# petercorke/robotics-toolbox-python

Measured on AMD Instinct MI355X. Metric: configurations/sec (Panda 7-DOF fkine+jacob0), higher is better.
Workload: dtype f64

## Files before the change

robotics-toolbox-python_amd/csrc/kin_kernels.hip:

```cpp
#include "kin_reg.h"
#include "diff_device.h"
#include "servo_device.h"
#include "diff_kernel.h"
#include <algorithm>
#include <cstring>

namespace rtbhip {

#ifndef RTB_T_PLAIN_MAX_BYTES
#define RTB_T_PLAIN_MAX_BYTES (136ll << 20)
#endif
constexpr long long kPoseCacheBytes = RTB_T_PLAIN_MAX_BYTES;
constexpr int kKinPosePlain = 1;
constexpr int kKinPacked = 2;

template <bool WANT_T, bool WANT_J, bool WANT_H, bool COALESCED, class S>
__device__ __forceinline__ void kin_tiles(KinParams kp, DevChain dc, const S *__restrict__ q, S *__restrict__ T, S *__restrict__ J,
                                          double *__restrict__ H, double *lds)
{
    double *rows = lds;
    double *qs = lds + kWave * kp.stride;
    const ConstChain ops = const_view(dc);
    const int lane = threadIdx.x;
    const int64_t tiles = (kp.N + kWave - 1) / kWave;
    const int W = 6 * kp.n;

    for (int64_t tile = blockIdx.x; tile < tiles; tile += gridDim.x) {
        const int64_t cfg0 = tile * kWave;
        const int64_t cfg = cfg0 + lane;
        const int64_t left = kp.N - cfg0;
        const int ncfg = left < kWave ? (int)left : kWave;
        const bool live = lane < ncfg;

        kin_load_q(kp, q, cfg, lane, qs);
        Pose P;
        kin_walk<(WANT_J || WANT_H)>(kp, ops, lane, qs, rows, P);
        if (WANT_H) kin_hessian(kp, lane, rows, live, H + cfg * (int64_t)(kp.n * W));
        if (WANT_T && WANT_J && !WANT_H && COALESCED && (kp.pad & kKinPacked)) {
            double *rowsT = qs + kWave * kp.qw;
            if (kp.has_base) pose_premul(P, kp.base);
            pose_store16(P, [&](int k, double v) { rowsT[lane * 17 + k] = v; });
            __syncthreads();
            kin_flush_packed(rowsT, rows, kp.stride, W, ncfg, T + cfg0 * (16 + W), lane);
            __syncthreads();
            continue;
        }
        if (WANT_J) {
            if (COALESCED) {
                __syncthreads();
                kin_flush(rows, kp.stride, W, ncfg, J + cfg0 * W, lane);
            } else {
                kin_store_own(rows, kp.stride, W, live, J + cfg * W, lane);
            }
        }
        if (WANT_T) {
            if (COALESCED) __syncthreads();
            kin_stage_T(kp, lane, rows, P);
            if (COALESCED) {
                __syncthreads();
                if (kp.pad & kKinPosePlain) kin_flush<false>(rows, kp.stride, 16, ncfg, T + cfg0 * 16, lane);
                else kin_flush<true>(rows, kp.stride, 16, ncfg, T + cfg0 * 16, lane);
            } else {
                kin_store_own(rows, kp.stride, 16, live, T + cfg * 16, lane);
            }
        }
        __syncthreads();
    }
}

template <bool WANT_T, bool WANT_J, bool WANT_H, bool COALESCED>
__global__ __launch_bounds__(kWave) void k_kin(KinParams kp, DevChain dc,
                                              const double *__restrict__ q, double *__restrict__ T,
                                              double *__restrict__ J, double *__restrict__ H)
{
    extern __shared__ __attribute__((aligned(16))) double lds[];
    kin_tiles<WANT_T, WANT_J, WANT_H, COALESCED>(kp, dc, q, T, J, H, lds);
}
template <bool WANT_T, bool WANT_J>
__global__ __launch_bounds__(kWave) void k_kin_f32(KinParams kp, DevChain dc, const float *__restrict__ q, float *__restrict__ T, float *__restrict__ J)
{
    extern __shared__ __attribute__((aligned(16))) double lds[];
    kin_tiles<WANT_T, WANT_J, false, true>(kp, dc, q, T, J, (double *)nullptr, lds);
}

#ifndef RTB_REG_WAVES
#define RTB_REG_WAVES 3
#endif
template <int NJ, bool WANT_T, bool WANT_J, bool PACKED = false, SegSig SIG = 0, class S>
__device__ __forceinline__ void reg_tile(const KinParams &kp, const ConstChain &cv, const S *__restrict__ q,
                                         S *__restrict__ T, S *__restrict__ J, double *buf, int lane,
                                         int64_t tile)
{
    constexpr int W = 6 * NJ;
    const int64_t cfg0 = tile * kWave;
    const int64_t left = kp.N - cfg0;
    const int ncfg = left < kWave ? (int)left : kWave;
    Pose P;
    double jac[6 * NJ];
    reg_compute<NJ, WANT_J, SIG>(kp, cv, q, cfg0 + lane, P, jac);
    if constexpr (PACKED) {
        static_assert(!PACKED || (WANT_T && WANT_J), "packed rows carry both");
        double *bufT = buf, *bufJ = buf + kPRound * 17;
#pragma unroll
        for (int r = 0; r < kWave / kPRound; ++r) {
            if (lane / kPRound == r) reg_stage_packed<NJ>(kp, P, jac, bufT, bufJ, lane % kPRound);
            __syncthreads();
            int rows = ncfg - r * kPRound;
            rows = rows < 0 ? 0 : (rows > kPRound ? kPRound : rows);
            kin_flush_packed(bufT, bufJ, W + 1, W, rows, T + (cfg0 + r * kPRound) * (16 + W), lane);
            __syncthreads();
        }
        return;
    }
    if (WANT_T) {
        reg_stage_T(kp, P, buf, lane);
        __syncthreads();
        if (kp.pad & kKinPosePlain) kin_flush<false>(buf, 17, 16, ncfg, T + cfg0 * 16, lane);
        else kin_flush<true>(buf, 17, 16, ncfg, T + cfg0 * 16, lane);
        __syncthreads();
    }
    if (WANT_J) {
#pragma unroll
        for (int r = 0; r < kWave / kJRound; ++r) {
            if (lane / kJRound == r) reg_stage_J<NJ>(jac, buf, lane % kJRound);
            __syncthreads();
            int rows = ncfg - r * kJRound;
            rows = rows < 0 ? 0 : (rows > kJRound ? kJRound : rows);
            kin_flush(buf, W + 1, W, rows, J + (cfg0 + r * kJRound) * W, lane);
            __syncthreads();
        }
    }
}

template <int NJ, bool WANT_T, bool WANT_J, bool PACKED = false, SegSig SIG = 0>
__global__ __launch_bounds__(kWave, (NJ <= kRegMaxJoints ? RTB_REG_WAVES : 2)) void k_kin_reg(KinParams kp, DevChain dc, const double *__restrict__ q,
                                                  double *__restrict__ T, double *__restrict__ J)
{
    extern __shared__ __attribute__((aligned(16))) double buf[];
    reg_tile<NJ, WANT_T, WANT_J, PACKED, SIG>(kp, const_view(dc), q, T, J, buf, threadIdx.x, xcd_tile());
}
template <int NJ, bool WANT_T, bool WANT_J, bool PACKED = false, SegSig SIG = 0>
__global__ __launch_bounds__(kWave, (NJ <= kRegMaxJoints ? RTB_REG_WAVES : 2)) void k_kin_reg_f32(KinParams kp, DevChain dc, const float *__restrict__ q,
                                                      float *__restrict__ T, float *__restrict__ J)
{
    extern __shared__ __attribute__((aligned(16))) double buf[];
    reg_tile<NJ, WANT_T, WANT_J, PACKED, SIG>(kp, const_view(dc), q, T, J, buf, threadIdx.x, xcd_tile());
}

static int g_hess_mode = 0;

template <int NJ>
__global__ __launch_bounds__(kWave, (NJ <= kRegMaxJoints ? 2 : 1)) void k_kin_hess(KinParams kp, DevChain dc, const double *__restrict__ q,
                                                       double *__restrict__ H)
{
    extern __shared__ __attribute__((aligned(16))) double buf[];
    const ConstChain cv = const_view(dc);
    const int lane = threadIdx.x;
    const int64_t cfg0 = (int64_t)blockIdx.x * kWave;
    const int64_t left = kp.N - cfg0;
    const int ncfg = left < kWave ? (int)left : kWave;
    constexpr int W = 6 * NJ;
    {
        Pose P;
        double jac[6 * NJ];
        reg_compute<NJ, true>(kp, cv, q, cfg0 + lane, P, jac);
        double *mine = buf + lane * (W + 1);
#pragma unroll
        for (int k = 0; k < W; ++k) mine[k] = jac[k];
    }
    __syncthreads();
    double *dst = H + cfg0 * (int64_t)(NJ * W);
    hessian_run<NJ>(buf, W + 1, ncfg, lane, [&](int f, double a, double b, bool both) {
        if (both) {
            typedef double v2d __attribute__((ext_vector_type(2)));
            v2d w = {a, b};
            __builtin_nontemporal_store(w, reinterpret_cast<v2d *>(dst + f));
        } else {
            __builtin_nontemporal_store(a, dst + f);
        }
    });
}

template <int NJ, int R>
__device__ __forceinline__ void hess_tile_emit(double (&jac)[6 * NJ], double *buf, int lane, int ncfg, double *__restrict__ Hrun)
{
    constexpr int HW = NJ * 6 * NJ, S = HW | 1, G = kWave / R;
    const int grp = lane / G;
    double *mine = buf + (lane - grp * G) * S;
    for (int r = 0; r < R; ++r) {
        const int cnt = ncfg - r * G < G ? ncfg - r * G : G;
        if (cnt <= 0) break;
        if (grp == r) {
#pragma unroll
            for (int k = 0; k < 6 * NJ; ++k) asm volatile("" : "+v"(jac[k]));
            hessian_from_jacobian(NJ, [&](int k) { return jac[k]; }, [&](int idx, double v) { mine[idx] = v; });
        }
        __syncthreads();
        double *dst = Hrun + (int64_t)(r * G) * HW;
        flush_rows<HW>(buf, S, cnt, lane, [&](int f, double a, double b) {
            typedef double v2d __attribute__((ext_vector_type(2)));
            v2d w = {a, b};
            __builtin_nontemporal_store(w, reinterpret_cast<v2d *>(dst + f));
        });
        __syncthreads();
    }
}

template <int NJ, int R>
__global__ __launch_bounds__(kWave, (NJ <= kRegMaxJoints && R >= 8 ? 2 : 1)) void k_kin_hess_tile(KinParams kp, DevChain dc, const double *__restrict__ q,
                                                                                               double *__restrict__ H)
{
    extern __shared__ __attribute__((aligned(16))) double buf[];
    const ConstChain cv = const_view(dc);
    const int lane = threadIdx.x;
    const int64_t cfg0 = (int64_t)blockIdx.x * kWave;
    const int64_t left = kp.N - cfg0;
    const int ncfg = left < kWave ? (int)left : kWave;
    Pose P;
    double jac[6 * NJ];
    reg_compute<NJ, true>(kp, cv, q, cfg0 + lane, P, jac);
    hess_tile_emit<NJ, R>(jac, buf, lane, ncfg, H + cfg0 * (int64_t)(NJ * 6 * NJ));
}
template <int NJ, int R>
static hipError_t launch_hess_tile(dim3 grid, hipStream_t s, const KinParams &kp, const DevChain &dc, const double *q, double *H)
{
    const size_t lds = (size_t)(kWave / R) * ((NJ * 6 * NJ) | 1) * sizeof(double);
    auto k = k_kin_hess_tile<NJ, R>;
    if (lds > 48 * 1024) { hipError_t e = hipFuncSetAttribute((const void *)k, hipFuncAttributeMaxDynamicSharedMemorySize, (int)lds); if (e != hipSuccess) return e; }
    hipLaunchKernelGGL(k, grid, dim3(kWave), lds, s, kp, dc, q, H);
    note_launch((int)grid.x, kWave, (int)lds);
    return hipGetLastError();
}
template <int NJ>
static hipError_t launch_hess_nj(dim3 grid, hipStream_t s, const KinParams &kp, const DevChain &dc, const double *q, double *H)
{
    if (g_hess_mode == 0) return launch_hess_tile<NJ, 4>(grid, s, kp, dc, q, H);
    if (g_hess_mode == 2) return launch_hess_tile<NJ, 8>(grid, s, kp, dc, q, H);
    const size_t lds = (size_t)kWave * (6 * NJ + 1) * sizeof(double);
    hipLaunchKernelGGL((k_kin_hess<NJ>), grid, dim3(kWave), lds, s, kp, dc, q, H);
    note_launch((int)grid.x, kWave, (int)lds);
    return hipGetLastError();
}

template <int NJ, int R>
__global__ __launch_bounds__(kWave, 1) void k_hess_from_jac(const double *__restrict__ J, int64_t N, double *__restrict__ H)
{
    extern __shared__ __attribute__((aligned(16))) double buf[];
    constexpr int W = 6 * NJ;
    const int lane = threadIdx.x;
    const int64_t cfg0 = (int64_t)blockIdx.x * kWave;
    const int64_t left = N - cfg0;
    const int ncfg = left < kWave ? (int)left : kWave;
    hj_load_tile(J + cfg0 * W, W, ncfg, buf, lane);
    __syncthreads();
    double jac[W];
    const double *mine = buf + lane * (W + 1);
#pragma unroll
    for (int k = 0; k < W; ++k) jac[k] = lane < ncfg ? mine[k] : 0.0;
    __syncthreads();
    hess_tile_emit<NJ, R>(jac, buf, lane, ncfg, H + cfg0 * (int64_t)(NJ * W));
}

__global__ __launch_bounds__(kWave) void k_hess_from_jac_any(int n, const double *__restrict__ J, int64_t N, double *__restrict__ H)
{
    const int64_t cfg = (int64_t)blockIdx.x * kWave + threadIdx.x;
    if (cfg >= N) return;
    const double *Jr = J + cfg * (int64_t)(6 * n);
    double *Hr = H + cfg * (int64_t)(6 * n * n);
    hessian_from_jacobian(n, [&](int k) { return Jr[k]; }, [&](int idx, double v) { Hr[idx] = v; });
}

template <int NJ>
static hipError_t launch_hess_from_jac_nj(dim3 grid, hipStream_t s, const double *J, int64_t N, double *H)
{
    constexpr int R = 4;
    const size_t a = (size_t)(kWave / R) * ((NJ * 6 * NJ) | 1), b = (size_t)kWave * (6 * NJ + 1);
    const size_t lds = (a > b ? a : b) * sizeof(double);
    auto k = k_hess_from_jac<NJ, R>;
    if (lds > 48 * 1024) { hipError_t e = hipFuncSetAttribute((const void *)k, hipFuncAttributeMaxDynamicSharedMemorySize, (int)lds); if (e != hipSuccess) return e; }
    hipLaunchKernelGGL(k, grid, dim3(kWave), lds, s, J, N, H);
    note_launch((int)grid.x, kWave, (int)lds);
// ... 296 lines not shown
    if (g_use_reg && c->n >= 1 && c->n <= kKinRegMax) {
        const size_t rl = (size_t)reg_lds_doubles_packed(c->n) * sizeof(double);
        const SegSig sig = kin_reg_sig(c, tool);
        hipError_t e = hipSuccess;
        switch (c->n) {
        case 1: e = launch_reg_packed<1>(grid, rl, s, kp, ops, q, TJ, sig); break;
        case 2: e = launch_reg_packed<2>(grid, rl, s, kp, ops, q, TJ, sig); break;
        case 3: e = launch_reg_packed<3>(grid, rl, s, kp, ops, q, TJ, sig); break;
        case 4: e = launch_reg_packed<4>(grid, rl, s, kp, ops, q, TJ, sig); break;
        case 5: e = launch_reg_packed<5>(grid, rl, s, kp, ops, q, TJ, sig); break;
        case 6: e = launch_reg_packed<6>(grid, rl, s, kp, ops, q, TJ, sig); break;
        case 7: e = launch_reg_packed<7>(grid, rl, s, kp, ops, q, TJ, sig); break;
        case 8: e = launch_reg_packed<8>(grid, rl, s, kp, ops, q, TJ, sig); break;
        case 9: e = launch_reg_packed<9>(grid, rl, s, kp, ops, q, TJ, sig); break;
        default: e = launch_reg_packed<10>(grid, rl, s, kp, ops, q, TJ, sig); break;
        }
        note_launch((int)grid.x, kWave, (int)rl);
        if (e != hipSuccess) return hip_fail(e, "k_kin_reg (packed) launch");
        return RTBHIP_OK;
    }
    const size_t lds = kin_lds_bytes(c->n, c->q_width) + (size_t)kWave * 17 * sizeof(double);
    if (lds > 160 * 1024) { set_error("chain too large for the per-wave LDS staging"); return RTBHIP_ELIMIT; }
    hipError_t e = launch_variant<true, true, false>(true, grid, lds, s, kp, ops, q, TJ, TJ, nullptr);
    note_launch((int)grid.x, kWave, (int)lds);
    if (e != hipSuccess) return hip_fail(e, "k_kin (packed) launch");
    return RTBHIP_OK;
}
int launch_kin_packed(const Chain *c, const DevChain &ops, const double *q, int64_t N, const Affine &base,
                      const Affine &tool, int frame, double *TJ, hipStream_t s)
{
    return launch_kin_packed_s(c, ops, q, N, base, tool, frame, TJ, s);
}
int launch_kin_packed_f32(const Chain *c, const DevChain &ops, const float *q, int64_t N, const Affine &base,
                          const Affine &tool, int frame, float *TJ, hipStream_t s)
{
    return launch_kin_packed_s(c, ops, q, N, base, tool, frame, TJ, s);
}

template <class S>
static int launch_kin_s(const Chain *c, const DevChain &ops, const S *q, int64_t N, const Affine &base,
                        const Affine &tool, int frame, S *T, S *J, double *H, hipStream_t s)
{
    constexpr bool kF64 = sizeof(S) == 8;
    if (N == 0) return RTBHIP_OK;
    KinParams kp;
    kp.n = c->n;
    kp.qw = c->q_width;
    kp.stride = kin_stride(c->n);
    kp.frame = frame;
    kp.has_base = base.used;
    kp.pad = (T && J && !H && (long long)N * 16 * (long long)sizeof(S) <= kPoseCacheBytes) ? kKinPosePlain : 0;
    kp.N = N;
    for (int i = 0; i < 12; i++) kp.base[i] = base.v[i];
    chain_tail(c, tool, kp.tail);
    const int64_t tiles = (N + kWave - 1) / kWave;
    int64_t g = (tiles + g_tiles_per_wave - 1) / g_tiles_per_wave;
    if (g > 0x7fffffff) g = 0x7fffffff;
    dim3 grid((unsigned)g);
    if constexpr (kF64) {
    if (g_use_reg && H && !T && !J && c->n >= 1 && c->n <= kKinRegMax && tiles <= 0x7fffffff) {
        grid = dim3((unsigned)tiles);
        hipError_t e = hipSuccess;
        switch (c->n) {
        case 1: e = launch_hess_nj<1>(grid, s, kp, ops, q, H); break;
        case 2: e = launch_hess_nj<2>(grid, s, kp, ops, q, H); break;
        case 3: e = launch_hess_nj<3>(grid, s, kp, ops, q, H); break;
        case 4: e = launch_hess_nj<4>(grid, s, kp, ops, q, H); break;
        case 5: e = launch_hess_nj<5>(grid, s, kp, ops, q, H); break;
        case 6: e = launch_hess_nj<6>(grid, s, kp, ops, q, H); break;
        case 7: e = launch_hess_nj<7>(grid, s, kp, ops, q, H); break;
        case 8: e = launch_hess_nj<8>(grid, s, kp, ops, q, H); break;
        case 9: e = launch_hess_nj<9>(grid, s, kp, ops, q, H); break;
        default: e = launch_hess_nj<10>(grid, s, kp, ops, q, H); break;
        }
        if (e != hipSuccess) return hip_fail(e, "k_kin_hess launch");
        return RTBHIP_OK;
    }
    }
    if (g_use_reg && !H && c->n >= 1 && c->n <= kKinRegMax && tiles <= 0x7fffffff) {
        grid = dim3((unsigned)tiles);
        const size_t rl = (size_t)(J ? reg_lds_doubles(c->n) : kWave * 17) * sizeof(double);
        const SegSig sig = kin_reg_sig(c, tool);
        hipError_t e = hipSuccess;
        switch (c->n) {
        case 1: e = launch_reg<1>(grid, rl, s, kp, ops, q, T, J, sig); break;
        case 2: e = launch_reg<2>(grid, rl, s, kp, ops, q, T, J, sig); break;
        case 3: e = launch_reg<3>(grid, rl, s, kp, ops, q, T, J, sig); break;
        case 4: e = launch_reg<4>(grid, rl, s, kp, ops, q, T, J, sig); break;
        case 5: e = launch_reg<5>(grid, rl, s, kp, ops, q, T, J, sig); break;
        case 6: e = launch_reg<6>(grid, rl, s, kp, ops, q, T, J, sig); break;
        case 7: e = launch_reg<7>(grid, rl, s, kp, ops, q, T, J, sig); break;
        case 8: e = launch_reg<8>(grid, rl, s, kp, ops, q, T, J, sig); break;
        case 9: e = launch_reg<9>(grid, rl, s, kp, ops, q, T, J, sig); break;
        default: e = launch_reg<10>(grid, rl, s, kp, ops, q, T, J, sig); break;
        }
        note_launch((int)grid.x, kWave, (int)rl);
        if (e != hipSuccess) return hip_fail(e, "k_kin_reg launch");
        return RTBHIP_OK;
    }
    const size_t lds = kin_lds_bytes(c->n, c->q_width);
    if (lds > 160 * 1024) { set_error("chain too large for the per-wave LDS staging"); return RTBHIP_ELIMIT; }
    const bool co = g_coalesced != 0;
    hipError_t e;
    const bool wt = T != nullptr, wj = J != nullptr, wh = H != nullptr;
    if (wt && wj && !wh) e = launch_variant<true, true, false>(co, grid, lds, s, kp, ops, q, T, J, H);
    else if (wt && !wj && !wh) e = launch_variant<true, false, false>(co, grid, lds, s, kp, ops, q, T, J, H);
    else if (!wt && wj && !wh) e = launch_variant<false, true, false>(co, grid, lds, s, kp, ops, q, T, J, H);
    else if (kF64 && !wt && !wj && wh) { if constexpr (kF64) e = launch_variant<false, false, true>(co, grid, lds, s, kp, ops, q, T, J, H); }
    else if (kF64 && wt && wj && wh) { if constexpr (kF64) e = launch_variant<true, true, true>(co, grid, lds, s, kp, ops, q, T, J, H); }
    else { set_error("launch_kin: unsupported output combination"); return RTBHIP_EINVAL; }
    note_launch((int)grid.x, kWave, (int)lds);
    if (e != hipSuccess) return hip_fail(e, "k_kin launch");
    return RTBHIP_OK;
}
int launch_kin(const Chain *c, const DevChain &ops, const double *q, int64_t N, const Affine &base,
               const Affine &tool, int frame, double *T, double *J, double *H, hipStream_t s)
{
    return launch_kin_s(c, ops, q, N, base, tool, frame, T, J, H, s);
}
int launch_kin_f32(const Chain *c, const DevChain &ops, const float *q, int64_t N, const Affine &base,
                   const Affine &tool, int frame, float *T, float *J, hipStream_t s)
{
    return launch_kin_s(c, ops, q, N, base, tool, frame, T, J, (double *)nullptr, s);
}

constexpr int kFleetMax = 32;
struct FleetArgs {
    FleetEntry e[kFleetMax];
    int32_t count, frame;
    int64_t tiles;
    int64_t tile_base;
};

template <int CLS, bool PACKED = false>
__global__ __launch_bounds__(kWave, (CLS == 0 ? RTB_REG_WAVES : 2)) void k_fleet(FleetArgs fa)
{
    extern __shared__ __attribute__((aligned(16))) double lds[];
    const int lane = threadIdx.x;
    const int64_t gt = (int64_t)blockIdx.x + fa.tile_base;
    int ci = 0;
    for (int i = 1; i < fa.count; ++i)
        if (gt >= fa.e[i].tile0) ci = i;
    const FleetEntry &fe = fa.e[ci];
    KinParams kp;
    kp.n = fe.n; kp.qw = fe.q_width; kp.stride = fe.stride;
    kp.frame = fa.frame; kp.has_base = 0; kp.pad = PACKED ? kKinPacked : 0; kp.N = fe.N;
    const ConstChain ops = const_view(fe.dc);
    for (int k = 0; k < 9; ++k) kp.tail[k] = ops.seg[fe.n].r[k];
    for (int k = 0; k < 3; ++k) kp.tail[9 + k] = ops.seg[fe.n].t[k];
    const int64_t local = gt - fe.tile0, ctiles = (fe.N + kWave - 1) / kWave;
    const int64_t tile = (ctiles <= 0x7fffffff) ? (int64_t)xcd_tile_of((unsigned)ctiles, (unsigned)local) : local;
    if (CLS == 0) {
        switch (fe.n) {
        case 1: reg_tile<1, true, true, PACKED>(kp, ops, fe.q, fe.T, fe.J, lds, lane, tile); return;
        case 2: reg_tile<2, true, true, PACKED>(kp, ops, fe.q, fe.T, fe.J, lds, lane, tile); return;
        case 3: reg_tile<3, true, true, PACKED>(kp, ops, fe.q, fe.T, fe.J, lds, lane, tile); return;
        case 4: reg_tile<4, true, true, PACKED>(kp, ops, fe.q, fe.T, fe.J, lds, lane, tile); return;
        case 5: reg_tile<5, true, true, PACKED>(kp, ops, fe.q, fe.T, fe.J, lds, lane, tile); return;
        case 6: reg_tile<6, true, true, PACKED>(kp, ops, fe.q, fe.T, fe.J, lds, lane, tile); return;
        case 7: reg_tile<7, true, true, PACKED>(kp, ops, fe.q, fe.T, fe.J, lds, lane, tile); return;
        default: reg_tile<8, true, true, PACKED>(kp, ops, fe.q, fe.T, fe.J, lds, lane, tile); return;
        }
    } else if (CLS == 1) {
        if (fe.n == 9) reg_tile<9, true, true, PACKED>(kp, ops, fe.q, fe.T, fe.J, lds, lane, tile);
        else reg_tile<10, true, true, PACKED>(kp, ops, fe.q, fe.T, fe.J, lds, lane, tile);
        return;
    }
    double *rows = lds;
    double *qs = lds + kWave * kp.stride;
    const int64_t cfg0 = tile * kWave, cfg = cfg0 + lane;
    const int64_t left = kp.N - cfg0;
    const int ncfg = left < kWave ? (int)left : kWave;
    const int W = 6 * kp.n;
    kin_load_q(kp, fe.q, cfg, lane, qs);
    Pose P;
    kin_walk<true>(kp, ops, lane, qs, rows, P);
    if (PACKED) {
        double *rowsT = qs + kWave * kp.qw;
        pose_store16(P, [&](int k, double v) { rowsT[lane * 17 + k] = v; });
        __syncthreads();
        kin_flush_packed(rowsT, rows, kp.stride, W, ncfg, fe.T + cfg0 * (16 + W), lane);
        return;
    }
    __syncthreads();
    kin_flush(rows, kp.stride, W, ncfg, fe.J + cfg0 * W, lane);
    __syncthreads();
    kin_stage_T(kp, lane, rows, P);
    __syncthreads();
    kin_flush(rows, kp.stride, 16, ncfg, fe.T + cfg0 * 16, lane);
}

static int fleet_class_of(int n) { return n <= kRegMaxJoints ? 0 : (n <= kKinRegMax ? 1 : 2); }
static int launch_fleet_class(int cls, const std::vector<FleetEntry> &entries, int frame, hipStream_t s, bool packed);
int launch_fleet(const std::vector<FleetEntry> &all, int frame, hipStream_t s, bool packed)
{
    std::vector<FleetEntry> by[3];
    for (const FleetEntry &e : all) by[fleet_class_of(e.n)].push_back(e);
    for (int c = 0; c < 3; ++c)
        if (!by[c].empty()) { int rc = launch_fleet_class(c, by[c], frame, s, packed); if (rc != RTBHIP_OK) return rc; }
    return RTBHIP_OK;
}

template <bool PACKED>
static void fleet_go(int cls, unsigned g, size_t lds, hipStream_t s, const FleetArgs &fa)
{
    if (cls == 0) hipLaunchKernelGGL((k_fleet<0, PACKED>), dim3(g), dim3(kWave), lds, s, fa);
    else if (cls == 1) hipLaunchKernelGGL((k_fleet<1, PACKED>), dim3(g), dim3(kWave), lds, s, fa);
    else hipLaunchKernelGGL((k_fleet<2, PACKED>), dim3(g), dim3(kWave), lds, s, fa);
}
template <bool PACKED>
static const void *fleet_fn(int cls)
{
    return cls == 0 ? (const void *)k_fleet<0, PACKED> : (cls == 1 ? (const void *)k_fleet<1, PACKED> : (const void *)k_fleet<2, PACKED>);
}

static int launch_fleet_class(int cls, const std::vector<FleetEntry> &entries, int frame, hipStream_t s, bool packed)
{
    for (size_t first = 0; first < entries.size(); first += kFleetMax) {
        FleetArgs fa;
        std::memset(&fa, 0, sizeof fa);
        fa.count = (int)std::min<size_t>(kFleetMax, entries.size() - first);
        fa.frame = frame;
        size_t lds = 0;
        int64_t tiles = 0;
        for (int i = 0; i < fa.count; i++) {
            fa.e[i] = entries[first + i];
            fa.e[i].stride = kin_stride(fa.e[i].n);
            fa.e[i].tile0 = tiles;
            tiles += (fa.e[i].N + kWave - 1) / kWave;
            lds = std::max(lds, cls < 2 ? (size_t)(packed ? reg_lds_doubles_packed(fa.e[i].n) : reg_lds_doubles(fa.e[i].n)) * sizeof(double)
                                        : kin_lds_bytes(fa.e[i].n, fa.e[i].q_width) + (packed ? (size_t)kWave * 17 * sizeof(double) : 0));
        }
        fa.tiles = tiles;
        if (lds > 160 * 1024) { set_error("fleet: chain too large for LDS staging"); return RTBHIP_ELIMIT; }
        const void *kfn = packed ? fleet_fn<true>(cls) : fleet_fn<false>(cls);
        if (lds > 48 * 1024) {
            hipError_t e = hipFuncSetAttribute(kfn, hipFuncAttributeMaxDynamicSharedMemorySize, (int)lds);
            if (e != hipSuccess) return hip_fail(e, "k_fleet attr");
        }
        for (int64_t t0 = 0; t0 < tiles; t0 += 0x7fffffff) {
            const int64_t g = std::min<int64_t>(0x7fffffff, tiles - t0);
            fa.tile_base = t0;
            if (packed) fleet_go<true>(cls, (unsigned)g, lds, s, fa); else fleet_go<false>(cls, (unsigned)g, lds, s, fa);
            note_launch((int)g, kWave, (int)lds);
            hipError_t e = hipGetLastError();
            if (e != hipSuccess) return hip_fail(e, "k_fleet launch");
        }
    }
    return RTBHIP_OK;
}

template <class G>
RTB_HD void vjp_pose_pullback(const Pose &P, int has_base, const double *base , G g , double (&w)[6])
{
#pragma clang fp contract(off)
    double h[12];
#pragma unroll
    for (int i = 0; i < 3; ++i)
#pragma unroll
        for (int c = 0; c < 4; ++c)
            h[4 * i + c] = has_base ? dot3x(base[i], g(c), base[4 + i], g(4 + c), base[8 + i], g(8 + c)) : g(4 * i + c);
    w[0] = h[3]; w[1] = h[7]; w[2] = h[11];
    w[3] = (mix_pm(P.r10, h[8], P.r20, h[4]) + mix_pm(P.r11, h[9], P.r21, h[5])) + mix_pm(P.r12, h[10], P.r22, h[6]);
    w[4] = (mix_pm(P.r20, h[0], P.r00, h[8]) + mix_pm(P.r21, h[1], P.r01, h[9])) + mix_pm(P.r22, h[2], P.r02, h[10]);
    w[5] = (mix_pm(P.r00, h[4], P.r10, h[0]) + mix_pm(P.r01, h[5], P.r11, h[1])) + mix_pm(P.r02, h[6], P.r12, h[2]);
}

template <bool WANT_GJ, class JGet, class GGet, class Acc>
RTB_HD void vjp_contract(int n, const double (&w)[6], JGet J, GGet G, Acc acc)
{
#pragma clang fp contract(off)
    if (!WANT_GJ) {
#pragma unroll
        for (int k = 0; k < n; ++k)
            acc(k, dot3x(J(k), w[0], J(n + k), w[1], J(2 * n + k), w[2]) + dot3x(J(3 * n + k), w[3], J(4 * n + k), w[4], J(5 * n + k), w[5]));
        return;
    }
    double sx = w[3], sy = w[4], sz = w[5];
#pragma unroll
    for (int k = n - 1; k >= 0; --k) {
        const double vx = J(k), vy = J(n + k), vz = J(2 * n + k), ox = J(3 * n + k), oy = J(4 * n + k), oz = J(5 * n + k);
        const double gvx = G(k), gvy = G(n + k), gvz = G(2 * n + k), gwx = G(3 * n + k), gwy = G(4 * n + k), gwz = G(5 * n + k);
        sx = sx + (mix_pm(vy, gvz, vz, gvy) + mix_pm(oy, gwz, oz, gwy));
        sy = sy + (mix_pm(vz, gvx, vx, gvz) + mix_pm(oz, gwx, ox, gwz));
        sz = sz + (mix_pm(vx, gvy, vy, gvx) + mix_pm(ox, gwy, oy, gwx));
        acc(k, dot3x(ox, sx, oy, sy, oz, sz));
    }
    double ax = w[0], ay = w[1], az = w[2];
#pragma unroll
    for (int k = 0; k < n; ++k) {
        const double ox = J(3 * n + k), oy = J(4 * n + k), oz = J(5 * n + k);
        const double gvx = G(k), gvy = G(n + k), gvz = G(2 * n + k);
        acc(k, dot3x(J(k), ax, J(n + k), ay, J(2 * n + k), az));
        ax = ax + mix_pm(gvy, oz, gvz, oy);
        ay = ay + mix_pm(gvz, ox, gvx, oz);
        az = az + mix_pm(gvx, oy, gvy, ox);
    }
}

template <class S>
RTB_HD void vjp_fill(const S *__restrict__ src, int W, int cnt, double *rows, int stride, int lane)
{
    const int total = cnt * W;
    int f = 2 * lane;
    int r = f / W, e = f - r * W;
    const int da = 128 / W, db = 128 - da * W;
    for (; f < total; f += 128) {
        double a, b;
#if defined(__HIP_DEVICE_COMPILE__)
        if constexpr (sizeof(S) == 4) {
            typedef float v2f __attribute__((ext_vector_type(2)));
            typedef v2f v2f_a4 __attribute__((aligned(4)));
            const v2f v = *reinterpret_cast<const v2f_a4 *>(src + f);
            a = v.x; b = v.y;
        } else {
            typedef double v2d __attribute__((ext_vector_type(2)));
            typedef v2d v2d_a8 __attribute__((aligned(8)));
            const v2d v = *reinterpret_cast<const v2d_a8 *>(src + f);
// ... 247 lines not shown
```

robotics-toolbox-python_amd/csrc/kin_reg.h:

```cpp
#pragma once
#include "kin_tile.h"
#include "trig.h"

namespace rtbhip {

constexpr int kRegMaxJoints = 8;
constexpr int kIkMaxJoints = 16;
constexpr int kKinRegMax = 10;
#ifndef RTB_JROUND
#define RTB_JROUND 32
#endif
constexpr int kJRound = RTB_JROUND;

RTB_HD int reg_lds_doubles(int n)
{
    const int a = kJRound * (6 * n + 1), b = kWave * 17;
    return a > b ? a : b;
}

#ifndef RTB_PROUND
#define RTB_PROUND 16
#endif
constexpr int kPRound = RTB_PROUND;
RTB_HD int reg_lds_doubles_packed(int n) { return kPRound * (17 + 6 * n + 1); }

inline SegSig chain_signature(const int32_t *jmeta, int n)
{
    if (n > 8) return 0;
    SegSig s = kSegSigPresent;
    for (int j = 0; j <= n; ++j) s |= seg_sig_of(j, jm_cls(jmeta[j]), jm_tmask(jmeta[j]));
    return s;
}
constexpr SegSig kSigPandaETS = kSegSigPresent | seg_sig_of(0, kSegIdentity, 4) | seg_sig_of(1, kSegRxN, 0) | seg_sig_of(2, kSegRxP, 6) | seg_sig_of(3, kSegRxP, 1) |
                                seg_sig_of(4, kSegRxN, 7) | seg_sig_of(5, kSegRxP, 0) | seg_sig_of(6, kSegRxP, 7) | seg_sig_of(7, kSegRz, 4);
constexpr SegSig kSigPandaURDF = kSegSigPresent | seg_sig_of(0, kSegIdentity, 4) | seg_sig_of(1, kSegRxN, 0) | seg_sig_of(2, kSegRxP, 2) | seg_sig_of(3, kSegRxP, 1) |
                                 seg_sig_of(4, kSegRxN, 3) | seg_sig_of(5, kSegRxP, 0) | seg_sig_of(6, kSegRxP, 1) | seg_sig_of(7, kSegRz, 4);
constexpr SegSig kSigUR = kSegSigPresent | seg_sig_of(0, kSegIdentity, 4) | seg_sig_of(1, kSegGeneral, 2) | seg_sig_of(2, kSegIdentity, 5) | seg_sig_of(3, kSegRzP, 1) |
                          seg_sig_of(4, kSegPermA, 4) | seg_sig_of(5, kSegPermB, 4) | seg_sig_of(6, kSegGeneral, 4);
template <SegSig SIG, int J, class CV>
RTB_HD void pose_mul_seg_by_sig(Pose &P, const CV &cv) { pose_mul_seg_sig<seg_sig_cls(SIG, J), seg_sig_tm(SIG, J)>(P, cv, J); }
template <int NJ, bool WANT_J, bool PLAIN, SegSig SIG, int J, class CV>
RTB_HD void reg_walk_step(const CV &cv, Pose &P, double (&jac)[6 * NJ], const int (&jmv)[NJ], const double (&c)[NJ], const double (&s)[NJ], const double (&d)[NJ])
{
    constexpr int j = J;
    {
#if defined(__HIP_DEVICE_COMPILE__)
        CV cvj = cv;
        if (PLAIN && SIG == 0 && cv_has_trig<CV>::value && j > 0) asm volatile("" : "+s"(cvj.seg), "+v"(P.tx));
        if (j == 0) pose_from_seg(P, cvj, 0);
        else if constexpr (SIG != 0) pose_mul_seg_by_sig<SIG, J>(P, cvj);
        else pose_mul_seg<((PLAIN && cv_has_trig<CV>::value) || cv_t3fma<CV>::value)>(P, cvj, j);
#else
        if (j == 0) pose_from_seg(P, cv, 0);
        else if constexpr (SIG != 0) pose_mul_seg_by_sig<SIG, J>(P, cv);
        else pose_mul_seg<cv_t3fma<CV>::value>(P, cv, j);
#endif
        if (WANT_J) {
            jac[j] = P.tx; jac[NJ + j] = P.ty; jac[2 * NJ + j] = P.tz;
            jac[3 * NJ + j] = P.r02; jac[4 * NJ + j] = P.r12; jac[5 * NJ + j] = P.r22;
        }
        if (jm_prismatic(jmv[j])) pose_tz(P, d[j]);
        else pose_rotz(P, c[j], s[j]);
        if (SIG == 0) sched_fence();
    }
}
template <int NJ, bool WANT_J, bool PLAIN, SegSig SIG, int J = 0, class CV>
RTB_HD void reg_walk_steps(const CV &cv, Pose &P, double (&jac)[6 * NJ], const int (&jmv)[NJ], const double (&c)[NJ], const double (&s)[NJ], const double (&d)[NJ])
{
    if constexpr (J < NJ) {
        reg_walk_step<NJ, WANT_J, PLAIN, SIG, J>(cv, P, jac, jmv, c, s, d);
        reg_walk_steps<NJ, WANT_J, PLAIN, SIG, J + 1>(cv, P, jac, jmv, c, s, d);
    }
}

template <int NJ, bool WANT_J>
RTB_HD void reg_close_jacobian(const Pose &P, int frame, const int (&jmv)[NJ], double (&jac)[6 * NJ])
{
    if (WANT_J) {
#pragma clang fp contract(off)
#pragma unroll
        for (int j = 0; j < NJ; ++j) {
            double zx = jac[3 * NJ + j], zy = jac[4 * NJ + j], zz = jac[5 * NJ + j];
            if (jm_flip(jmv[j])) { zx = -zx; zy = -zy; zz = -zz; }
            double vx, vy, vz, wx, wy, wz;
            if (jm_prismatic(jmv[j])) {
                vx = zx; vy = zy; vz = zz;
                wx = 0.0; wy = 0.0; wz = 0.0;
            } else {
                const double dx = P.tx - jac[j], dy = P.ty - jac[NJ + j], dz = P.tz - jac[2 * NJ + j];
                vx = mix_pm(zy, dz, zz, dy); vy = mix_pm(zz, dx, zx, dz); vz = mix_pm(zx, dy, zy, dx);
                wx = zx; wy = zy; wz = zz;
            }
            if (frame == 1) {
                double a = vx, b = vy, e = vz;
                vx = dot3x(P.r00, a, P.r10, b, P.r20, e);
                vy = dot3x(P.r01, a, P.r11, b, P.r21, e);
                vz = dot3x(P.r02, a, P.r12, b, P.r22, e);
                a = wx; b = wy; e = wz;
                wx = dot3x(P.r00, a, P.r10, b, P.r20, e);
                wy = dot3x(P.r01, a, P.r11, b, P.r21, e);
                wz = dot3x(P.r02, a, P.r12, b, P.r22, e);
            }
            jac[j] = vx; jac[NJ + j] = vy; jac[2 * NJ + j] = vz;
            jac[3 * NJ + j] = wx; jac[4 * NJ + j] = wy; jac[5 * NJ + j] = wz;
        }
    }
}

template <int NJ, bool WANT_J, bool PLAIN = false, SegSig SIG = 0, class CV, class TL>
RTB_HD void reg_core(const CV &cv, TL tail , int frame, const double (&qv)[NJ], Pose &P,
                     double (&jac)[6 * NJ])
{
    static_assert(SIG == 0 || (PLAIN && NJ <= 8), "a structure signature goes with the straight-line walk");
    double c[NJ], s[NJ], d[NJ];
    int jmv[NJ];
    bool big = false;
#pragma unroll
    for (int j = 0; j < NJ; ++j) {
        jmv[j] = PLAIN ? 0 : cv.jmeta[j];
        d[j] = PLAIN ? qv[j] : qv[j] * (jm_flip(jmv[j]) ? -1.0 : 1.0);
    }
#pragma unroll
    for (int j = 0; j < NJ; ++j) {
        if constexpr (cv_has_trig<CV>::value) sincos_reduced_tab(d[j], s[j], c[j], cv.trig);
        else sincos_reduced(d[j], s[j], c[j]);
        big = big || !(fabs(d[j]) < kTrigFastLimit);
    }
    if (wave_any(big)) {
#pragma unroll
        for (int j = 0; j < NJ; ++j) sincos(d[j], &s[j], &c[j]);
    }
    reg_walk_steps<NJ, WANT_J, PLAIN, SIG>(cv, P, jac, jmv, c, s, d);
    if constexpr (SIG != 0) pose_mul_seg_by_sig<SIG, NJ>(P, cv);
    else pose_mul_general<((PLAIN && cv_has_trig<CV>::value) || cv_t3fma<CV>::value)>(P, [&](int k) { return tail[k]; });
    sched_fence();
    reg_close_jacobian<NJ, WANT_J>(P, frame, jmv, jac);
}

template <int NJ, bool WANT_J, SegSig SIG = 0, class CV, class S>
RTB_HD void reg_compute(const KinParams &kp, const CV &cv, const S *__restrict__ q, int64_t cfg,
                        Pose &P, double (&jac)[6 * NJ])
{
    const bool live = cfg < kp.N;
    double qv[NJ];
    if constexpr (SIG != 0) {
        const S *qrow = q + (live ? cfg : 0) * kp.qw;
        int jq[NJ];
#pragma unroll
        for (int j = 0; j < NJ; ++j) jq[j] = jm_jq(cv.jmeta[j]);
#pragma unroll
        for (int j = 0; j < NJ; ++j) qv[j] = qrow[jq[j]];
#pragma unroll
        for (int j = 0; j < NJ; ++j) qv[j] = live ? qv[j] : 0.0;
        reg_core<NJ, WANT_J, true, SIG>(cv, &cv.seg[NJ].r[0], kp.frame, qv, P, jac);
    } else {
        const S *qrow = q + cfg * kp.qw;
#pragma unroll
        for (int j = 0; j < NJ; ++j) qv[j] = live ? qrow[jm_jq(cv.jmeta[j])] : 0.0;
        reg_core<NJ, WANT_J>(cv, kp.tail, kp.frame, qv, P, jac);
    }
}

template <int NJ>
RTB_HD void reg_stage_J(const double (&jac)[6 * NJ], double *buf, int slot_lane)
{
    double *mine = buf + slot_lane * (6 * NJ + 1);
#pragma unroll
    for (int k = 0; k < 6 * NJ; ++k) mine[k] = jac[k];
}

template <int NJ>
RTB_HD void reg_stage_packed(const KinParams &kp, Pose P, const double (&jac)[6 * NJ], double *bufT, double *bufJ, int slot_lane)
{
    if (kp.has_base) pose_premul(P, kp.base);
    double *mt = bufT + slot_lane * 17;
    pose_store16(P, [&](int k, double v) { mt[k] = v; });
    double *mj = bufJ + slot_lane * (6 * NJ + 1);
#pragma unroll
    for (int k = 0; k < 6 * NJ; ++k) mj[k] = jac[k];
}

RTB_HD void reg_stage_T(const KinParams &kp, Pose P, double *buf, int lane)
{
    if (kp.has_base) pose_premul(P, kp.base);
    double *mine = buf + lane * 17;
    pose_store16(P, [&](int k, double v) { mine[k] = v; });
}

}
```

robotics-toolbox-python_amd/csrc/kin_tile.h:

```cpp
#pragma once
#include "kin_device.h"

namespace rtbhip {

struct KinParams {
    int32_t n, qw, stride, frame;
    int32_t has_base, pad;
    int64_t N;
    double base[12];
    double tail[12];
};

RTB_HD int kin_stride(int n)
{
    int s = 6 * n;
    if (s < 16) s = 16;
    return s + 1;
}
RTB_HD size_t kin_lds_bytes(int n, int qw) { return (size_t)kWave * (kin_stride(n) + qw) * sizeof(double); }

template <class S>
RTB_HD void kin_load_q(const KinParams &kp, const S *__restrict__ q, int64_t cfg, int lane,
                       double *qs)
{
    const bool live = cfg < kp.N;
    const S *src = q + cfg * kp.qw;
    int c = 0;
    for (; c + 4 <= kp.qw; c += 4) {
        double a0 = live ? src[c] : 0.0, a1 = live ? src[c + 1] : 0.0;
        double a2 = live ? src[c + 2] : 0.0, a3 = live ? src[c + 3] : 0.0;
        qs[(c + 0) * kWave + lane] = a0;
        qs[(c + 1) * kWave + lane] = a1;
        qs[(c + 2) * kWave + lane] = a2;
        qs[(c + 3) * kWave + lane] = a3;
    }
    for (; c < kp.qw; ++c) qs[c * kWave + lane] = live ? src[c] : 0.0;
}

template <bool WANT_J, class CV>
RTB_HD void kin_walk(const KinParams &kp, const CV &cv, int lane, const double *qs, double *rows, Pose &P)
{
    double *mine = rows + lane * kp.stride;
    chain_walk<WANT_J>(cv, kp.n, kp.tail, P,
                       [&](int c) { return qs[c * kWave + lane]; },
                       [&](int slot, double v) { mine[slot] = v; });
    if (WANT_J)
        jacobian_close(cv, kp.n, P, kp.frame, [&](int s) { return mine[s]; },
                       [&](int s, double v) { mine[s] = v; });
}

RTB_HD void kin_stage_T(const KinParams &kp, int lane, double *rows, Pose P)
{
    if (kp.has_base) pose_premul(P, kp.base);
    double *mine = rows + lane * kp.stride;
    pose_store16(P, [&](int k, double v) { mine[k] = v; });
}


template <bool NT>
RTB_HD void store_pair_f32(float *__restrict__ dst, double a, double b)
{
#if defined(__HIP_DEVICE_COMPILE__)
    typedef float v2f __attribute__((ext_vector_type(2)));
    typedef v2f v2f_a4 __attribute__((aligned(4)));
    v2f w = {(float)a, (float)b};
    if (NT) __builtin_nontemporal_store(w, reinterpret_cast<v2f_a4 *>(dst));
    else *reinterpret_cast<v2f_a4 *>(dst) = w;
#else
    dst[0] = (float)a;
    dst[1] = (float)b;
#endif
}

template <bool NT = true, class S>
RTB_HD void kin_flush(const double *rows, int stride, int W, int ncfg, S *__restrict__ dst,
                      int lane)
{
    const int total = ncfg * W;
    int f = 2 * lane;
    int cfg = f / W, e = f - cfg * W;
    const int da = 128 / W, db = 128 - da * W;
    for (; f < total; f += 128) {
        const double *src = rows + cfg * stride + e;
        if constexpr (sizeof(S) == 4) {
            store_pair_f32<NT>(dst + f, src[0], src[1]);
            e += db;
            cfg += da;
            if (e >= W) { e -= W; cfg += 1; }
            continue;
        }
        double2 v;
        v.x = src[0];
        v.y = src[1];
#if defined(__HIP_DEVICE_COMPILE__)
        if (NT) {
            typedef double v2d __attribute__((ext_vector_type(2)));
            v2d w = {v.x, v.y};
            __builtin_nontemporal_store(w, reinterpret_cast<v2d *>(dst + f));
        } else {
            *reinterpret_cast<double2 *>(dst + f) = v;
        }
#else
        *reinterpret_cast<double2 *>(dst + f) = v;
#endif
        e += db;
        cfg += da;
        if (e >= W) { e -= W; cfg += 1; }
    }
}

template <bool NT = true, class S>
RTB_HD void kin_flush_packed(const double *rowsT, const double *rowsJ, int strideJ, int W, int ncfg, S *__restrict__ dst, int lane)
{
    const int PW = 16 + W;
    const int total = ncfg * PW;
    int f = 2 * lane;
    int cfg = f / PW, e = f - cfg * PW;
    const int da = 128 / PW, db = 128 - da * PW;
    for (; f < total; f += 128) {
        const double *src = e < 16 ? rowsT + cfg * 17 + e : rowsJ + cfg * strideJ + (e - 16);
        if constexpr (sizeof(S) == 4) {
            store_pair_f32<NT>(dst + f, src[0], src[1]);
            e += db;
            cfg += da;
            if (e >= PW) { e -= PW; cfg += 1; }
            continue;
        }
        double2 v;
        v.x = src[0];
        v.y = src[1];
#if defined(__HIP_DEVICE_COMPILE__)
        if (NT) {
            typedef double v2d __attribute__((ext_vector_type(2)));
            v2d w = {v.x, v.y};
            __builtin_nontemporal_store(w, reinterpret_cast<v2d *>(dst + f));
        } else {
            *reinterpret_cast<double2 *>(dst + f) = v;
        }
#else
        *reinterpret_cast<double2 *>(dst + f) = v;
#endif
        e += db;
        cfg += da;
        if (e >= PW) { e -= PW; cfg += 1; }
    }
}

#if defined(__HIPCC__)
__device__ __forceinline__ void flush_run(const double *rows, int stride, int W, int ncfg, double *__restrict__ dst, int lane)
{
    const int total = ncfg * W;
    for (int f = 2 * lane; f < total; f += 2 * kWave) {
        const int r = f / W, e = f - r * W;
        const double a = rows[r * stride + e];
        if (f + 1 < total) {
            const double b = (e + 1 < W) ? rows[r * stride + e + 1] : rows[(r + 1) * stride];
            typedef double v2d __attribute__((ext_vector_type(2)));
            v2d w = {a, b};
            __builtin_nontemporal_store(w, reinterpret_cast<v2d *>(dst + f));
        } else {
            __builtin_nontemporal_store(a, dst + f);
        }
    }
}
#endif

template <class S>
RTB_HD void kin_store_own(const double *rows, int stride, int W, bool live, S *__restrict__ dst_row,
                          int lane)
{
    if (!live) return;
    const double *mine = rows + lane * stride;
    for (int e = 0; e < W; e += 2) {
        if constexpr (sizeof(S) == 4) {
            store_pair_f32<false>(dst_row + e, mine[e], mine[e + 1]);
            continue;
        }
        double2 v;
        v.x = mine[e];
        v.y = mine[e + 1];
        *reinterpret_cast<double2 *>(dst_row + e) = v;
    }
}

RTB_HD void kin_hessian(const KinParams &kp, int lane, const double *rows, bool live,
                        double *__restrict__ Hrow)
{
    if (!live) return;
    const double *mine = rows + lane * kp.stride;
    hessian_from_jacobian(kp.n, [&](int s) { return mine[s]; }, [&](int idx, double v) { Hrow[idx] = v; });
}

}
```

Before: 13.17 billion.

## Software-pipeline LDS flushes for full tiles and prefetch chain constants into SGPRs

Adds a compile-time-sized flush path for full tiles. It issues LDS reads a few pieces ahead of the nontemporal global stores, so load latency overlaps with the stores. For signature-specialised chains it also fetches the needed segment constants in two halves into pinned scalar registers before walking the joints, and touches the constant block early to warm the scalar cache. This costs SGPR pressure, more code size, and extra template instantiations. The fleet path opts out with PIPE=0.

```diff
diff --git a/robotics-toolbox-python_amd/csrc/kin_kernels.hip b/robotics-toolbox-python_amd/csrc/kin_kernels.hip
--- a/robotics-toolbox-python_amd/csrc/kin_kernels.hip
+++ b/robotics-toolbox-python_amd/csrc/kin_kernels.hip
@@ -86,7 +86,7 @@
 #ifndef RTB_REG_WAVES
 #define RTB_REG_WAVES 3
 #endif
-template <int NJ, bool WANT_T, bool WANT_J, bool PACKED = false, SegSig SIG = 0, class S>
+template <int NJ, bool WANT_T, bool WANT_J, bool PACKED = false, SegSig SIG = 0, int PIPE = 1, class S>
 __device__ __forceinline__ void reg_tile(const KinParams &kp, const ConstChain &cv, const S *__restrict__ q,
                                          S *__restrict__ T, S *__restrict__ J, double *buf, int lane,
                                          int64_t tile)
@@ -107,7 +107,7 @@
             __syncthreads();
             int rows = ncfg - r * kPRound;
             rows = rows < 0 ? 0 : (rows > kPRound ? kPRound : rows);
-            kin_flush_packed(bufT, bufJ, W + 1, W, rows, T + (cfg0 + r * kPRound) * (16 + W), lane);
+            kin_flush_packed<true, PIPE * kPRound, W>(bufT, bufJ, W + 1, W, rows, T + (cfg0 + r * kPRound) * (16 + W), lane);
             __syncthreads();
         }
         return;
@@ -115,8 +115,8 @@
     if (WANT_T) {
         reg_stage_T(kp, P, buf, lane);
         __syncthreads();
-        if (kp.pad & kKinPosePlain) kin_flush<false>(buf, 17, 16, ncfg, T + cfg0 * 16, lane);
-        else kin_flush<true>(buf, 17, 16, ncfg, T + cfg0 * 16, lane);
+        if (kp.pad & kKinPosePlain) kin_flush<false, PIPE * kWave, 16>(buf, 17, 16, ncfg, T + cfg0 * 16, lane);
+        else kin_flush<true, PIPE * kWave, 16>(buf, 17, 16, ncfg, T + cfg0 * 16, lane);
         __syncthreads();
     }
     if (WANT_J) {
@@ -126,7 +126,7 @@
             __syncthreads();
             int rows = ncfg - r * kJRound;
             rows = rows < 0 ? 0 : (rows > kJRound ? kJRound : rows);
-            kin_flush(buf, W + 1, W, rows, J + (cfg0 + r * kJRound) * W, lane);
+            kin_flush<true, PIPE * kJRound, W>(buf, W + 1, W, rows, J + (cfg0 + r * kJRound) * W, lane);
             __syncthreads();
         }
     }
@@ -729,18 +729,18 @@
     const int64_t tile = (ctiles <= 0x7fffffff) ? (int64_t)xcd_tile_of((unsigned)ctiles, (unsigned)local) : local;
     if (CLS == 0) {
         switch (fe.n) {
-        case 1: reg_tile<1, true, true, PACKED>(kp, ops, fe.q, fe.T, fe.J, lds, lane, tile); return;
-        case 2: reg_tile<2, true, true, PACKED>(kp, ops, fe.q, fe.T, fe.J, lds, lane, tile); return;
-        case 3: reg_tile<3, true, true, PACKED>(kp, ops, fe.q, fe.T, fe.J, lds, lane, tile); return;
-        case 4: reg_tile<4, true, true, PACKED>(kp, ops, fe.q, fe.T, fe.J, lds, lane, tile); return;
-        case 5: reg_tile<5, true, true, PACKED>(kp, ops, fe.q, fe.T, fe.J, lds, lane, tile); return;
-        case 6: reg_tile<6, true, true, PACKED>(kp, ops, fe.q, fe.T, fe.J, lds, lane, tile); return;
-        case 7: reg_tile<7, true, true, PACKED>(kp, ops, fe.q, fe.T, fe.J, lds, lane, tile); return;
-        default: reg_tile<8, true, true, PACKED>(kp, ops, fe.q, fe.T, fe.J, lds, lane, tile); return;
+        case 1: reg_tile<1, true, true, PACKED, 0, 0>(kp, ops, fe.q, fe.T, fe.J, lds, lane, tile); return;
+        case 2: reg_tile<2, true, true, PACKED, 0, 0>(kp, ops, fe.q, fe.T, fe.J, lds, lane, tile); return;
+        case 3: reg_tile<3, true, true, PACKED, 0, 0>(kp, ops, fe.q, fe.T, fe.J, lds, lane, tile); return;
+        case 4: reg_tile<4, true, true, PACKED, 0, 0>(kp, ops, fe.q, fe.T, fe.J, lds, lane, tile); return;
+        case 5: reg_tile<5, true, true, PACKED, 0, 0>(kp, ops, fe.q, fe.T, fe.J, lds, lane, tile); return;
+        case 6: reg_tile<6, true, true, PACKED, 0, 0>(kp, ops, fe.q, fe.T, fe.J, lds, lane, tile); return;
+        case 7: reg_tile<7, true, true, PACKED, 0, 0>(kp, ops, fe.q, fe.T, fe.J, lds, lane, tile); return;
+        default: reg_tile<8, true, true, PACKED, 0, 0>(kp, ops, fe.q, fe.T, fe.J, lds, lane, tile); return;
         }
     } else if (CLS == 1) {
-        if (fe.n == 9) reg_tile<9, true, true, PACKED>(kp, ops, fe.q, fe.T, fe.J, lds, lane, tile);
-        else reg_tile<10, true, true, PACKED>(kp, ops, fe.q, fe.T, fe.J, lds, lane, tile);
+        if (fe.n == 9) reg_tile<9, true, true, PACKED, 0, 0>(kp, ops, fe.q, fe.T, fe.J, lds, lane, tile);
+        else reg_tile<10, true, true, PACKED, 0, 0>(kp, ops, fe.q, fe.T, fe.J, lds, lane, tile);
         return;
     }
     double *rows = lds;
diff --git a/robotics-toolbox-python_amd/csrc/kin_reg.h b/robotics-toolbox-python_amd/csrc/kin_reg.h
--- a/robotics-toolbox-python_amd/csrc/kin_reg.h
+++ b/robotics-toolbox-python_amd/csrc/kin_reg.h
@@ -64,12 +64,12 @@
         if (SIG == 0) sched_fence();
     }
 }
-template <int NJ, bool WANT_J, bool PLAIN, SegSig SIG, int J = 0, class CV>
+template <int NJ, bool WANT_J, bool PLAIN, SegSig SIG, int J = 0, int JEND = NJ, class CV>
 RTB_HD void reg_walk_steps(const CV &cv, Pose &P, double (&jac)[6 * NJ], const int (&jmv)[NJ], const double (&c)[NJ], const double (&s)[NJ], const double (&d)[NJ])
 {
-    if constexpr (J < NJ) {
+    if constexpr (J < JEND) {
         reg_walk_step<NJ, WANT_J, PLAIN, SIG, J>(cv, P, jac, jmv, c, s, d);
-        reg_walk_steps<NJ, WANT_J, PLAIN, SIG, J + 1>(cv, P, jac, jmv, c, s, d);
+        reg_walk_steps<NJ, WANT_J, PLAIN, SIG, J + 1, JEND>(cv, P, jac, jmv, c, s, d);
     }
 }
 
@@ -107,6 +107,83 @@
     }
 }
 
+template <int NJ>
+struct SigSegs {
+    DevSeg seg[NJ + 1];
+    const int32_t *jmeta;
+};
+constexpr bool sig_reads_entry(SegSig sig, int j, int k )
+{
+    const int cls = seg_sig_cls(sig, j), tm = seg_sig_tm(sig, j);
+    if (j == 0 || cls == kSegGeneral || ((RTB_SIG_UNFUSED_GENERAL >> cls) & 1)) return true;
+    return k < 9 ? seg_kind(cls, k) == kCA : ((tm >> (k - 9)) & 1) != 0;
+}
+constexpr int sig_reads_count(SegSig sig, int j0, int j1, int k1 = 0)
+{
+    int m = 0;
+    for (int a = j0; a <= j1; ++a)
+        for (int b = 0; b < (a < j1 ? 12 : k1); ++b) m += sig_reads_entry(sig, a, b) ? 1 : 0;
+    return m;
+}
+constexpr int kSigFetchMax = 40;
+constexpr int sig_split(SegSig sig, int nj)
+{
+    int h = 1;
+    while (h <= nj && 2 * sig_reads_count(sig, 0, h) < sig_reads_count(sig, 0, nj + 1)) ++h;
+    return h;
+}
+constexpr bool sig_fetches(SegSig sig, int nj)
+{
+    if (sig == 0 || nj > 8) return false;
+    const int h = sig_split(sig, nj);
+    return sig_reads_count(sig, 0, nj + 1) <= kSigFetchMax && sig_reads_count(sig, 0, h) <= 30 && sig_reads_count(sig, h, nj + 1) <= 30;
+}
+template <int V> struct IntC { static constexpr int v = V; };
+template <SegSig SIG, int J0, int J1, int I = 12 * J0, class F>
+RTB_HD void sig_each(F f)
+{
+    if constexpr (I < 12 * J1) {
+        if constexpr (sig_reads_entry(SIG, I / 12, I % 12)) f(IntC<I / 12>(), IntC<I % 12>(), IntC<sig_reads_count(SIG, J0, I / 12, I % 12)>());
+        sig_each<SIG, J0, J1, I + 1>(f);
+    }
+}
+template <SegSig SIG, int NJ, int J0, int J1, class CV>
+RTB_HD void sig_fetch(const CV &cv, SigSegs<NJ> &cs)
+{
+    static_assert(!cv_fused_translation<CV>::value, "the unfused views' reading pattern");
+    sig_each<SIG, J0, J1>([&](auto j, auto k, auto) {
+        if constexpr (k.v < 9) cs.seg[j.v].r[k.v] = cv.seg[j.v].r[k.v];
+        else cs.seg[j.v].t[k.v - 9] = cv.seg[j.v].t[k.v - 9];
+    });
+#if defined(__HIP_DEVICE_COMPILE__)
+    constexpr int m = sig_reads_count(SIG, J0, J1);
+    static_assert(m >= 1 && m <= 30, "one statement's operands");
+    double v[m];
+    sig_each<SIG, J0, J1>([&](auto j, auto k, auto slot) {
+        if constexpr (k.v < 9) v[slot.v] = cs.seg[j.v].r[k.v];
+        else v[slot.v] = cs.seg[j.v].t[k.v - 9];
+    });
+#define RTB_PIN(i) "s"(v[(i) < m ? (i) : m - 1])
+    sched_fence();
+    asm volatile("" ::RTB_PIN(0), RTB_PIN(1), RTB_PIN(2), RTB_PIN(3), RTB_PIN(4), RTB_PIN(5), RTB_PIN(6), RTB_PIN(7), RTB_PIN(8), RTB_PIN(9), RTB_PIN(10),
+                 RTB_PIN(11), RTB_PIN(12), RTB_PIN(13), RTB_PIN(14), RTB_PIN(15), RTB_PIN(16), RTB_PIN(17), RTB_PIN(18), RTB_PIN(19), RTB_PIN(20),
+                 RTB_PIN(21), RTB_PIN(22), RTB_PIN(23), RTB_PIN(24), RTB_PIN(25), RTB_PIN(26), RTB_PIN(27), RTB_PIN(28), RTB_PIN(29));
+    sched_fence();
+#undef RTB_PIN
+#endif
+}
+#if defined(__HIP_DEVICE_COMPILE__)
+template <int NJ, class CV>
+__device__ __forceinline__ void sig_touch(const CV &cv)
+{
+    const auto *w = (const __attribute__((address_space(4))) int32_t *)cv.seg;
+    int any = 0;
+#pragma unroll
+    for (int b = 0; b < (NJ + 1) * (int)sizeof(DevSeg); b += 64) any |= w[b / 4];
+    asm volatile("" ::"s"(any));
+}
+#endif
+
 template <int NJ, bool WANT_J, bool PLAIN = false, SegSig SIG = 0, class CV, class TL>
 RTB_HD void reg_core(const CV &cv, TL tail , int frame, const double (&qv)[NJ], Pose &P,
                      double (&jac)[6 * NJ])
@@ -129,6 +206,18 @@
     if (wave_any(big)) {
 #pragma unroll
         for (int j = 0; j < NJ; ++j) sincos(d[j], &s[j], &c[j]);
+    }
+    if constexpr (sig_fetches(SIG, NJ) && !cv_fused_translation<CV>::value) {
+        constexpr int H = sig_split(SIG, NJ), E = H >= 2 ? H - 2 : 0;
+        SigSegs<NJ> cs = {};
+        sig_fetch<SIG, NJ, 0, H>(cv, cs);
+        reg_walk_steps<NJ, WANT_J, PLAIN, SIG, 0, E>(cs, P, jac, jmv, c, s, d);
+        if constexpr (H <= NJ) sig_fetch<SIG, NJ, H, NJ + 1>(cv, cs);
+        reg_walk_steps<NJ, WANT_J, PLAIN, SIG, E, NJ>(cs, P, jac, jmv, c, s, d);
+        pose_mul_seg_by_sig<SIG, NJ>(P, cs);
+        sched_fence();
+        reg_close_jacobian<NJ, WANT_J>(P, frame, jmv, jac);
+        return;
     }
     reg_walk_steps<NJ, WANT_J, PLAIN, SIG>(cv, P, jac, jmv, c, s, d);
     if constexpr (SIG != 0) pose_mul_seg_by_sig<SIG, NJ>(P, cv);
@@ -150,6 +239,9 @@
         for (int j = 0; j < NJ; ++j) jq[j] = jm_jq(cv.jmeta[j]);
 #pragma unroll
         for (int j = 0; j < NJ; ++j) qv[j] = qrow[jq[j]];
+#if defined(__HIP_DEVICE_COMPILE__)
+        if constexpr (!cv_fused_translation<CV>::value) sig_touch<NJ>(cv);
+#endif
 #pragma unroll
         for (int j = 0; j < NJ; ++j) qv[j] = live ? qv[j] : 0.0;
         reg_core<NJ, WANT_J, true, SIG>(cv, &cv.seg[NJ].r[0], kp.frame, qv, P, jac);
diff --git a/robotics-toolbox-python_amd/csrc/kin_tile.h b/robotics-toolbox-python_amd/csrc/kin_tile.h
--- a/robotics-toolbox-python_amd/csrc/kin_tile.h
+++ b/robotics-toolbox-python_amd/csrc/kin_tile.h
@@ -72,10 +72,58 @@
 #endif
 }
 
-template <bool NT = true, class S>
+#if defined(__HIP_DEVICE_COMPILE__)
+constexpr int kFlushGroup = 3;
+template <bool NT, class S>
+__device__ __forceinline__ void store_piece(S *__restrict__ dst, double a, double b)
+{
+    if constexpr (sizeof(S) == 4) {
+        store_pair_f32<NT>(dst, a, b);
+    } else {
+        typedef double v2d __attribute__((ext_vector_type(2)));
+        v2d w = {a, b};
+        if (NT) __builtin_nontemporal_store(w, reinterpret_cast<v2d *>(dst));
+        else *reinterpret_cast<v2d *>(dst) = w;
+    }
+}
+template <bool NT, int TOTAL, class S, class Src>
+__device__ __forceinline__ void flush_full(S *__restrict__ dst, int lane, Src src_of)
+{
+    static_assert(TOTAL > 0 && TOTAL % 2 == 0, "whole pairs");
+    constexpr int NP = (TOTAL + 127) / 128;
+    double a[kFlushGroup], b[kFlushGroup];
+    if (NT) asm volatile("");
+    auto has = [&](int p) { return 128 * (p + 1) <= TOTAL || 2 * lane + 128 * p < TOTAL; };
+    auto read = [&](int p) {
+        if (has(p)) {
+            const double *src = src_of(2 * lane + 128 * p);
+            a[p % kFlushGroup] = src[0];
+            b[p % kFlushGroup] = src[1];
+        }
+    };
+#pragma unroll
+    for (int p = 0; p < kFlushGroup && p < NP; ++p) read(p);
+#pragma unroll
+    for (int p = 0; p < NP; ++p) {
+        if (has(p)) store_piece<NT>(dst + 2 * lane + 128 * p, a[p % kFlushGroup], b[p % kFlushGroup]);
+        if (p + kFlushGroup < NP) read(p + kFlushGroup);
+    }
+    if (NT) asm volatile("");
+}
+#endif
+
+template <bool NT = true, int FULL_ROWS = 0, int FULL_W = 0, class S>
 RTB_HD void kin_flush(const double *rows, int stride, int W, int ncfg, S *__restrict__ dst,
                       int lane)
 {
+#if defined(__HIP_DEVICE_COMPILE__)
+    if constexpr (FULL_ROWS > 0) {
+        if (ncfg == FULL_ROWS) {
+            flush_full<NT, FULL_ROWS * FULL_W>(dst, lane, [&](int f) { const int cfg = (unsigned)f / (unsigned)FULL_W; return rows + cfg * stride + (f - cfg * FULL_W); });
+            return;
+        }
+    }
+#endif
     const int total = ncfg * W;
     int f = 2 * lane;
     int cfg = f / W, e = f - cfg * W;
@@ -109,9 +157,20 @@
     }
 }
 
-template <bool NT = true, class S>
+template <bool NT = true, int FULL_ROWS = 0, int FULL_W = 0, class S>
 RTB_HD void kin_flush_packed(const double *rowsT, const double *rowsJ, int strideJ, int W, int ncfg, S *__restrict__ dst, int lane)
 {
+#if defined(__HIP_DEVICE_COMPILE__)
+    if constexpr (FULL_ROWS > 0) {
+        if (ncfg == FULL_ROWS) {
+            flush_full<NT, FULL_ROWS * (16 + FULL_W)>(dst, lane, [&](int f) {
+                const int cfg = (unsigned)f / (unsigned)(16 + FULL_W), e = f - cfg * (16 + FULL_W);
+                return e < 16 ? rowsT + cfg * 17 + e : rowsJ + cfg * strideJ + (e - 16);
+            });
+            return;
+        }
+    }
+#endif
     const int PW = 16 + W;
     const int total = ncfg * PW;
     int f = 2 * lane;
```

After: 13.59 billion (median of 6 runs). 1.03x the previous value.
